# charlie-foxtrot/RTLSDR-Airband

Measured on NVIDIA H100. Metric: iq_msamples_per_s_fft_demod, higher is better.
Workload: dtype f32

## Files before the change

### rtlsdr-airband_b200/csrc/abg_internal.h

```cpp
#pragma once
#include <cuda_runtime.h>
#include <stdint.h>

#include <mutex>

struct AbgPerDeviceSize {
    std::mutex m;
    size_t v[64] = {};
    template <class F>
    cudaError_t ensure(size_t want, F&& apply) {
        int dev = 0;
        cudaGetDevice(&dev);
        dev &= 63;
        std::lock_guard<std::mutex> lock(m);
        if (want > v[dev]) {
            cudaError_t e = apply();
            if (e != cudaSuccess) return e;
            v[dev] = want;
        }
        return cudaSuccess;
    }
};

#define ABG_AGC_EXTRA 100
#define ABG_SQ_BUF 102
#define ABG_MAX_TONES 52

enum { SQ_CLOSED = 0, SQ_OPENING = 1, SQ_CLOSING = 2, SQ_LOW_SIGNAL_ABORT = 3, SQ_OPEN = 4 };

struct ChanParams {
    int32_t dev;
    int32_t modulation;
    int32_t needs_raw_iq, has_iq_outputs;
    uint32_t dm_dphi;
    float alpha, ampfactor;
    int32_t afc;
    int32_t notch_on;
    float nd0, nd1, nd2;
    int32_t lp_on;
    float lp_gain, lp_yc0, lp_yc1;
    int32_t ctcss_on;
    int32_t n_tones[2];
    int32_t window[2];
};

struct ChanState {
    float noise_floor;
    int32_t manual;
    float manual_level, normal_ratio, flappy_ratio, avg_cap;
    float pre_full, pre_capped, post_full, post_capped;
    float level_cache;
    int32_t using_post;
    int32_t next_state, cur_state, delay;
    uint32_t sample_count_mod16;
    int32_t low_signal_count;
    uint32_t recent_open_count, closed_sample_count;
    int32_t head;
    unsigned long long open_count, flappy_count;
    int32_t ct_enough[2], ct_count[2], ct_has_tone[2];
    unsigned long long ct_found[2], ct_not_found[2];
    float nx1, nx2, ny1, ny2;
    float lx1r, lx1i, lx2r, lx2i, ly1r, ly1i, ly2r, ly2i;
    float agcavgfast;
    uint32_t dm_phi;
    float pr, pj, prev_waveout;
    unsigned long long active_counter;
    int32_t axc_prev;
};

struct K1Dev {
    const unsigned char* raw;
    unsigned long long start_byte;
    int32_t n_frames;
    int32_t pos0;
    int32_t g0, n_channels;
    int32_t hop_bytes;
    int32_t sfmt;
    float2* spec;
    int32_t spec_first_pos;
    int32_t wave_batch;
};

struct K2Dev {
    int32_t n_batches;
    int32_t fft_size;
    const float2* spec;
};

struct K1Launch {
    int fft_size;
    int n_devices;
    int max_frames;
    int frames_per_tile;
    int tile_bytes_cap;
    const K1Dev* devs;
    const int32_t* bins;
    const float* window_scaled;
    const float2* tw1;
    const float2* tw2;
    float* win;
    float2* iqin;
    int Gp;
    int sfmt;
};
cudaError_t abg_launch_k1(const K1Launch& L, cudaStream_t s);
int abg_k1_tile_frames(int fft_size, int sfmt, int hop_bytes, int* tile_bytes_cap);
cudaError_t abg_launch_k1_pruned(const K1Launch& L, const float2* twn, int max_channels, cudaStream_t s);
int abg_k1p_tile_frames(int fft_size, int sfmt, int hop_bytes, int max_channels, int* tile_bytes_cap);

struct K1TcPlan {
    int eligible;
    int K, HC, S, NC, ND, C2p, KBS, NSTB, acc_regs, smem_bytes, halo, consumer_warpgroups;
    int pps;
    size_t table_bytes;
};
struct K1TcTables {
    const int32_t* tab_of_dev;
    const signed char* btab;
    const long long* sq;
    int* counter;
    int32_t* status;
    double cscale;
};
int abg_k1tc_plan(int fft_size, int sfmt, int hop_bytes, int max_channels, int digits, K1TcPlan* p);
void abg_k1tc_build_table(const K1TcPlan& p, int fft_size, int sfmt, const float* wsc, const int32_t* bins, int n_channels, signed char* tab,
                          long long* sq, double* cscale);
cudaError_t abg_launch_k1_tc(const K1Launch& L, const K1TcPlan& p, const K1TcTables& T, int sm_count, cudaStream_t s);
int abg_k1tc_trace_dump(long long* out);

#define ABG_SPEC_FPC 32
struct SpecCfg {
    const float* wsc;
    float* partial;
    int32_t* counter;
    float* ring;
    int32_t hop_bytes, sfmt, stride, n_sel, n_chunks, ring_cap;
};
struct SpecRun {
    const unsigned char* raw;
    unsigned long long first_byte;
    int32_t n_batches;
    int32_t ring_pos0;
};
struct SpecArgs {
    const SpecCfg* cfg;
    const SpecRun* run;
    const float2* tw1;
    const float2* tw2;
    int wave_batch;
};
cudaError_t abg_launch_spectrum(int fft_size, const SpecArgs& a, int n_devices, int max_items, cudaStream_t s);

struct CarCfg {
    float* ring;
    int32_t g0, n_channels, ring_cap;
};
struct CarRun {
    int32_t n_batches;
    int32_t ring_pos0;
};
struct CarArgs {
    const CarCfg* cfg;
    const CarRun* run;
    const float2* iqin;
    int Gp, wave_batch;
};
cudaError_t abg_launch_carrier(const CarArgs& a, int n_devices, int max_items, cudaStream_t s);
int abg_carrier_items(int n_channels);

struct InmCfg {
    unsigned char* ring;
    uint32_t* hist;
    int32_t* counter;
    long long* partial;
    int32_t sfmt, hop_bytes, n_chunks, ring_cap;
    float scale;
};
#define ABG_INM_PARTIAL 6
struct InmRun {
    const unsigned char* raw;
    unsigned long long first_byte;
    int32_t n_batches;
    int32_t ring_pos0;
};
struct InmArgs {
    const InmCfg* cfg;
    const InmRun* run;
    int wave_batch;
};
cudaError_t abg_launch_input_meter(const InmArgs& a, int n_devices, int max_items, cudaStream_t s);
int abg_input_meter_chunks(int batch_bytes);

struct K2Launch {
    int G, Gp, P, wave_batch, fm_demod, iq_stride;
    int lanes_per_warp;
    int nfm_blocks;
    const ChanParams* params;
    ChanState* state;
    const K2Dev* devs;
    int32_t* bins;
    const int32_t* base_bins;
    float* win;
    float2* iqin;
    float* win_next;
    float2* iqin_next;
    float* wout;
    float2* iqout;
    float* sqbuf;
    const float* tone_coeff;
    float* tone_q1;
    float* tone_q2;
    float* tone_mag;
    unsigned char* axc;
    const float* sincos_lut;
};
cudaError_t abg_launch_k2(const K2Launch& L, cudaStream_t s);
int abg_k2_stats_dump(unsigned long long* out);

struct MixInput {
    int32_t g;
    int32_t dev;
    float mult_l, mult_r;
};
struct MixLaunch {
    int n_mixers, n_batches, wave_batch, P, Gp;
    const int32_t* offsets;
    const MixInput* inputs;
    const K2Dev* devs;
    const float* wout;
    const unsigned char* axc;
    float* sums;
    int32_t* flags;
    float* host_sums;
    int32_t* host_flags;
};
cudaError_t abg_launch_mix(const MixLaunch& L, cudaStream_t s);
struct K2Export {
    float* host_wout;
    float2* host_iqout;
    unsigned char* host_axc;
    size_t stride;
};
cudaError_t abg_launch_k2_tail(const K2Launch& L, const K2Export& X, cudaStream_t s);
```

### rtlsdr-airband_b200/csrc/k1_tc.cu

```cuda
#include <cuda_runtime.h>
#include <math.h>
#include <stdint.h>
#include <stdlib.h>

#include <algorithm>

#include "../../include/airband_b200.h"
#include "abg_internal.h"
#include "tc_ptx.cuh"

namespace {
using namespace tc;
extern long long* g_tc_trace;

constexpr int TC_THREADS = 384;
constexpr int TC_A_THREADS = 96;
constexpr int TC_CONSUMER_WARPS = 8;
constexpr int TC_CTRL_BYTES = 1024;
constexpr int TC_MAX_STAGES = 32;
constexpr int TC_INFO_SLOTS = 4;

struct TileInfo {
    const unsigned char* src;
    int nf;
    int pos;
    int gbase;
    int nch;
    int tab;
    int pad;
};

struct TcArgs {
    const K1Dev* devs;
    const int32_t* tab_of_dev;
    const signed char* btab;
    const long long* sq;
    float* win;
    float2* iqin;
    int* counter;
    int32_t* status;
    double cscale;
    int Gp, n_devices, tiles_per_dev, total_tiles;
    int K, hop_bytes, S, npairs;
    int KBS, NSTG, pps;
    int a_bytes, stage_bytes;
    long long* trace;
};

struct Ctrl {
    unsigned long long full[TC_MAX_STAGES], empty[TC_MAX_STAGES];
    unsigned long long info_full[TC_INFO_SLOTS], info_empty[TC_INFO_SLOTS];
    TileInfo info[TC_INFO_SLOTS];
};
static_assert(sizeof(Ctrl) <= TC_CTRL_BYTES, "control block too large");

struct StageSeq {
    int p, np, q0, nq, nk, sh, mk;
    __device__ __forceinline__ void start(const TcArgs& a) {
        nk = (a.K - 32 * p + a.hop_bytes - 1) / a.hop_bytes;
        q0 = 0;
        nq = min(a.KBS, nk);
        np = min(min(a.pps, a.npairs - p), ((a.K - (nk - 1) * a.hop_bytes + 31) >> 5) - p);
        sh = np > 1 ? nq - 1 : 31;
        mk = np > 1 ? nq - 1 : -1;
    }
    __device__ __forceinline__ void first(const TcArgs& a) {
        p = 0;
        start(a);
    }
    __device__ __forceinline__ bool next(const TcArgs& a) {
        q0 += nq;
        if (q0 < nk) {
            nq = min(a.KBS, nk - q0);
            return true;
        }
        p += np;
        if (p >= a.npairs) return false;
        start(a);
        return true;
    }
};

template <int ND, int C2P, bool S8, bool GROUPED>
__global__ void __launch_bounds__(TC_THREADS, 1) k1_tc_kernel(const TcArgs a) {
    constexpr int NCOL = (ND * C2P + 31) & ~31;
    constexpr int KSTEP_BYTES = NCOL * 32;
    extern __shared__ __align__(1024) unsigned char smem[];
    Ctrl* c = reinterpret_cast<Ctrl*>(smem);
    const uint32_t ring = smem_u32(smem + TC_CTRL_BYTES);
    const uint32_t full0 = smem_u32(&c->full[0]), empty0 = smem_u32(&c->empty[0]);
    const int tid = threadIdx.x, lane = tid & 31;
    const int warp = __shfl_sync(0xffffffffu, tid >> 5, 0);

    if (tid == 0) {
        for (int i = 0; i < TC_MAX_STAGES; i++) {
            mbar_init(smem_u32(&c->full[i]), TC_A_THREADS + 1);
            mbar_init(smem_u32(&c->empty[i]), TC_CONSUMER_WARPS);
        }
        for (int i = 0; i < TC_INFO_SLOTS; i++) {
            mbar_init(smem_u32(&c->info_full[i]), 1);
            mbar_init(smem_u32(&c->info_empty[i]), TC_CONSUMER_WARPS);
        }
        fence_mbar_init();
    }
    __syncthreads();

#define TC_TRACE_STAGE(role, it, st, e)                                                                          \
    do {                                                                                                         \
        if (a.trace && (it) == 3 && (st) < 16) a.trace[((size_t)blockIdx.x * 4 + (role)) * 64 + 32 + 2 * (st) + (e)] = clock64(); \
    } while (0)
#define TC_TRACE(role, it, ev)                                                                                   \
    do {                                                                                                         \
        if (a.trace && (it) < 8 && (threadIdx.x & 31) == 0) a.trace[(((size_t)blockIdx.x * 4 + (role)) * 16 + (it)) * 4 + (ev)] = clock64(); \
    } while (0)
    if (warp < 3) {
        const int rr = tid & 7;
        uint32_t stg = 0, ph = 0;
        for (int it = 0;; ++it) {
            const int slot = it & (TC_INFO_SLOTS - 1);
            mbar_wait_spin(smem_u32(&c->info_full[slot]), (it / TC_INFO_SLOTS) & 1);
            const TileInfo ti = c->info[slot];
            if (ti.nf <= 0) break;
            if (warp == 0) TC_TRACE(0, it, 0);
            const int valid = (ti.nf - 1) * a.hop_bytes + a.K;
            StageSeq u;
            u.first(a);
            do {
                mbar_wait_spin(empty0 + 8 * stg, ph ^ 1);
                const int first = u.q0 * a.hop_bytes + 32 * u.p;
                const unsigned char* src = ti.src + first;
                const int rem = valid - first, nrows = 127 + u.nq, ncol = 2 * u.np;
                const uint32_t dst = ring + stg * (uint32_t)a.stage_bytes;
                const int total = ((nrows + 7) >> 3) * 8 * ncol;
                for (int i = tid; i - tid < total; i += TC_A_THREADS) {
                    const int u8 = i >> 3, rb = u8 / ncol, c = u8 - rb * ncol, r = rb * 8 + rr, off = r * a.hop_bytes + 16 * c;
                    if (i < total && r < nrows && off < rem) cp_async16(dst + c * a.S + r * 16, src + off);
                }
                cp_async_arrive_noinc(full0 + 8 * stg);
                if (++stg == (uint32_t)a.NSTG) stg = 0, ph ^= 1;
            } while (u.next(a));
            if (warp == 0) TC_TRACE(0, it, 3);
        }
    } else if (warp == 3) {
        const uint32_t leader = elect_one();
        const size_t tab_bytes = (size_t)a.K * NCOL;
        const int ks_per_row = a.hop_bytes / 32;
        auto publish = [&](int it) -> int {
            const int slot = it & (TC_INFO_SLOTS - 1);
            mbar_wait_spin(smem_u32(&c->info_empty[slot]), ((it / TC_INFO_SLOTS) & 1) ^ 1);
            TileInfo ti{};
            ti.nf = 0;
            ti.tab = -1;
            for (;;) {
                const int t = atomicAdd(a.counter, 1);
                if (t >= a.total_tiles) break;
                const int dev = t / a.tiles_per_dev, st = t - dev * a.tiles_per_dev;
                const K1Dev dv = a.devs[dev];
                const int f0 = st * 128;
                if (f0 >= dv.n_frames || dv.n_channels <= 0) continue;
                ti.src = dv.raw + dv.start_byte + (unsigned long long)f0 * dv.hop_bytes;
                ti.nf = min(128, dv.n_frames - f0);
                ti.pos = dv.pos0 + f0;
                ti.gbase = dv.g0;
                ti.nch = dv.n_channels;
                ti.tab = a.tab_of_dev[dev];
                break;
            }
            c->info[slot] = ti;
            mbar_arrive(smem_u32(&c->info_full[slot]));
            return ti.tab;
        };
        uint32_t stg = 0, ph = 0;
        int tab = lane == 0 ? publish(0) : 0;
        tab = __shfl_sync(0xffffffffu, tab, 0);
        for (int it = 0; tab >= 0; ++it) {
            int next_tab = lane == 0 ? publish(it + 1) : 0;
            next_tab = __shfl_sync(0xffffffffu, next_tab, 0);
            const signed char* src = a.btab + (size_t)tab * tab_bytes;
            TC_TRACE(2, it, 0);
            StageSeq u;
            u.first(a);
            int st = 0;
            do {
                mbar_wait_spin(empty0 + 8 * stg, ph ^ 1);
                TC_TRACE_STAGE(2, it, st, 0);
                if (leader) {
                    const uint32_t bar = full0 + 8 * stg, dst = ring + stg * (uint32_t)a.stage_bytes + (uint32_t)a.a_bytes;
                    mbar_arrive_expect_tx(bar, (uint32_t)(u.np * u.nq * KSTEP_BYTES));
                    for (int g = 0; g < u.np; g++)
                        for (int q = 0; q < u.nq; q++)
                            bulk_g2s(dst + (g * u.nq + q) * KSTEP_BYTES, src + (size_t)((u.q0 + q) * ks_per_row + u.p + g) * KSTEP_BYTES,
                                     (uint32_t)KSTEP_BYTES, bar);
                }
                TC_TRACE_STAGE(2, it, st, 1);
                st++;
                if (++stg == (uint32_t)a.NSTG) stg = 0, ph ^= 1;
            } while (u.next(a));
            TC_TRACE(2, it, 1);
            tab = next_tab;
        }
    } else if (warp >= 4) {
        const int wg = (warp - 4) >> 2;
        const int wq = warp & 3;
        uint32_t acc[NCOL / 2];
        const uint64_t adesc0 = smem_desc_noswizzle(0, (uint32_t)a.S, 128u), bdesc0 = smem_desc_noswizzle(0, (uint32_t)NCOL * 16u, 128u);
        const uint64_t a_hi = adesc0 >> 32 << 32, b_hi = bdesc0 >> 32 << 32;
        const uint32_t a_lo0 = (uint32_t)adesc0 + (ring >> 4) + (uint32_t)(wg * 64);
        const uint32_t b_lo0 = (uint32_t)bdesc0 + ((ring + (uint32_t)a.a_bytes) >> 4);
        const uint32_t stage16 = (uint32_t)a.stage_bytes >> 4, pair16 = (uint32_t)a.S >> 3;
        uint32_t stg = 0, ph = 0, prev_empty = 0;
        for (int it = 0;; ++it) {
            const int slot = it & (TC_INFO_SLOTS - 1);
            mbar_wait_spin(smem_u32(&c->info_full[slot]), (it / TC_INFO_SLOTS) & 1);
            const TileInfo ti = c->info[slot];
            if (ti.nf <= 0) break;
            if (warp == 4) TC_TRACE(3, it, 0);
            StageSeq u;
            u.first(a);
            uint32_t accumulate = 0;
            int st = 0;
            wgmma_fence_regs(acc);
            do {
                mbar_wait_spin(full0 + 8 * stg, ph);
                fence_proxy_async();
                if (warp == 4) TC_TRACE_STAGE(3, it, st, 0);
                const uint32_t a_lo = a_lo0 + stg * stage16, b_lo = b_lo0 + stg * stage16;
                const int n_mma = GROUPED ? u.np * u.nq : u.nq;
                for (int j = 0; j < n_mma; j++) {
                    const uint32_t a_off = GROUPED ? (uint32_t)(j >> u.sh) * pair16 + (uint32_t)(j & u.mk) : (uint32_t)j;
                    wgmma_fence_regs(acc);
                    wgmma_fence();
                    WgmmaI8<NCOL, S8>::mma(acc, a_hi | (a_lo + a_off), b_hi | (b_lo + j * (KSTEP_BYTES >> 4)), accumulate);
                    wgmma_commit();
                    wgmma_fence_regs(acc);
                    accumulate = 1;
                }
                wgmma_wait_groups(n_mma);
                mbar_arrive_if(prev_empty, st > 0 && lane == 0);
                prev_empty = empty0 + 8 * stg;
                if (warp == 4) TC_TRACE_STAGE(3, it, st, 1);
                st++;
                if (++stg == (uint32_t)a.NSTG) stg = 0, ph ^= 1;
            } while (u.next(a));
            wgmma_wait<0>();
            wgmma_fence_regs(acc);
            if (lane == 0) mbar_arrive(prev_empty);
            if (warp == 4) TC_TRACE(1, it, 1);
            constexpr long long MUL = S8 ? 1 : 2, OFF = S8 ? 0 : 255;
            const int r0 = wg * 64 + wq * 16 + (lane >> 2);
            const long long* sq = a.sq + (size_t)ti.tab * C2P;
#pragma unroll
            for (int jb = 0; jb < C2P / 8; jb++) {
                const int ch = 4 * jb + (lane & 3);
                const long long sq_re = __ldg(sq + 2 * ch), sq_im = __ldg(sq + 2 * ch + 1);
#pragma unroll
                for (int h = 0; h < 2; h++) {
                    long long v[2];
#pragma unroll
                    for (int e = 0; e < 2; e++) {
                        v[e] = 0;
#pragma unroll
                        for (int d = 0; d < ND; d++) v[e] = (v[e] << 8) + (long long)(int32_t)acc[4 * (d * C2P / 8 + jb) + 2 * h + e];
                    }
                    const float xr = (float)((double)(MUL * v[0] - OFF * sq_re) * a.cscale);
                    const float xi = (float)((double)(MUL * v[1] - OFF * sq_im) * a.cscale);
                    const int row = r0 + 8 * h;
                    if (row < ti.nf && ch < ti.nch) {
                        const size_t o = (size_t)(ti.pos + row) * a.Gp + ti.gbase + ch;
                        a.win[o] = sqrtf(__fadd_rn(__fmul_rn(xr, xr), __fmul_rn(xi, xi)));
                        a.iqin[o] = make_float2(xr, xi);
                    }
                }
            }
            __syncwarp();
            if (lane == 0) mbar_arrive(smem_u32(&c->info_empty[slot]));
            if (warp == 4) TC_TRACE(1, it, 2);
        }
    }
}

template <int ND, int C2P, bool S8>
cudaError_t tc_launch_one(const TcArgs& args, int grid, size_t smem, cudaStream_t s) {
    auto kern = args.pps > 1 ? k1_tc_kernel<ND, C2P, S8, true> : k1_tc_kernel<ND, C2P, S8, false>;
    static AbgPerDeviceSize configured[2];
    cudaError_t e = configured[args.pps > 1].ensure(smem, [&]() {
        cudaError_t e2 = cudaFuncSetAttribute(kern, cudaFuncAttributeMaxDynamicSharedMemorySize, (int)smem);
        if (e2 != cudaSuccess) return e2;
        cudaFuncSetAttribute(kern, cudaFuncAttributePreferredSharedMemoryCarveout, cudaSharedmemCarveoutMaxShared);
        return cudaSuccess;
    });
    if (e != cudaSuccess) return e;
    kern<<<grid, TC_THREADS, smem, s>>>(args);
    return cudaGetLastError();
}
template <int ND, bool S8>
cudaError_t tc_launch_nd(const TcArgs& args, int C2p, int grid, size_t smem, cudaStream_t s) {
    switch (C2p) {
        case 8: return tc_launch_one<ND, 8, S8>(args, grid, smem, s);
        case 16: return tc_launch_one<ND, 16, S8>(args, grid, smem, s);
        case 24: return tc_launch_one<ND, 24, S8>(args, grid, smem, s);
        case 32: return tc_launch_one<ND, 32, S8>(args, grid, smem, s);
        case 40: return tc_launch_one<ND, 40, S8>(args, grid, smem, s);
        case 48: return tc_launch_one<ND, 48, S8>(args, grid, smem, s);
        case 56: return tc_launch_one<ND, 56, S8>(args, grid, smem, s);
        case 64: return tc_launch_one<ND, 64, S8>(args, grid, smem, s);
    }
    return cudaErrorInvalidValue;
}

long long* g_tc_trace = nullptr;
}

int abg_k1tc_trace_dump(long long* out) {
    if (!g_tc_trace) return -1;
    cudaDeviceSynchronize();
    return cudaMemcpy(out, g_tc_trace, sizeof(long long) * 256 * 4 * 16 * 4, cudaMemcpyDeviceToHost) == cudaSuccess ? 0 : -1;
}

int abg_k1tc_plan(int fft_size, int sfmt, int hop_bytes, int max_channels, int digits, K1TcPlan* p) {
    *p = K1TcPlan{};
    if (sfmt != ABG_SFMT_U8 && sfmt != ABG_SFMT_S8) return 0;
    if (hop_bytes % 32 != 0 || hop_bytes < 32) return 0;
    if (digits != 3 && digits != 4) return 0;
    const int K = fft_size * 2;
    const int HC = hop_bytes / 16;
    const int halo = (K - 32) / hop_bytes;
    int rows = 128 + halo;
    if ((rows & 1) == 0) rows++;
    const int S = rows * 16;
    const int C2p = (2 * max_channels + 7) & ~7;
    const int NC = (digits * C2p + 31) & ~31;
    if (NC > 256) return 0;
    if (K > 16384) return 0;
    const size_t kstep = (size_t)NC * 32;
    size_t cap = 200 * 1024;
    if (const char* ev = getenv("ABG_K1_TC_CAP_KB")) cap = std::min<size_t>(227, std::max(64, atoi(ev))) * 1024;
    int max_stages = TC_MAX_STAGES;
    if (const char* ev = getenv("ABG_K1_TC_STAGES")) max_stages = std::min(TC_MAX_STAGES, std::max(2, atoi(ev)));
    const size_t hard_cap = 227 * 1024;
    auto stage_bytes = [&](int pps, int kbs) { return (((size_t)2 * pps * S + 127) & ~(size_t)127) + (size_t)pps * kbs * kstep; };
    auto stages = [&](int pps, int kbs, size_t c) {
        return c > TC_CTRL_BYTES ? (int)std::min<size_t>(max_stages, (c - TC_CTRL_BYTES) / stage_bytes(pps, kbs)) : 0;
    };
    const int kq = (K + hop_bytes - 1) / hop_bytes, npairs = std::min(HC / 2, K / 32);
    int pps = kq <= 2 ? std::max(1, std::min(12 / kq, npairs)) : 1, kbs = kq;
    while (pps > 1 && stages(pps, kbs, cap) < 4) pps--;
    while (kbs > 1 && stages(pps, kbs, cap) < 4) kbs = (kbs + 1) / 2;
    int nst = stages(pps, kbs, cap);
    if (nst < 2) nst = stages(pps, kbs, hard_cap);
    if (nst < 2) return 0;
    p->pps = pps;
    p->eligible = 1; p->K = K; p->HC = HC; p->S = S; p->NC = NC; p->ND = digits; p->C2p = C2p; p->KBS = kbs; p->NSTB = nst;
    p->acc_regs = NC / 2;
    p->consumer_warpgroups = 2;
    p->smem_bytes = (int)(TC_CTRL_BYTES + (size_t)nst * stage_bytes(pps, kbs)); p->halo = halo;
    p->table_bytes = (size_t)K * NC;
    return 1;
}

void abg_k1tc_build_table(const K1TcPlan& p, int fft_size, int sfmt, const float* wsc, const int32_t* bins, int n_channels, signed char* tab,
                          long long* sq, double* cscale) {
    const int N = fft_size, K = p.K, NC = p.NC, ND = p.ND;
    double gmax = 0.0;
    for (int n = 0; n < N; n++) gmax = std::max(gmax, fabs((double)wsc[n]));
    if (gmax <= 0.0) gmax = 1.0;
    const double Q = ldexp(1.0, 8 * ND - 2);
    std::fill(tab, tab + (size_t)K * NC, (signed char)0);
    for (int o = 0; o < p.C2p; o++) sq[o] = 0;
    for (int c = 0; c < n_channels; c++) {
        const int b = bins[c] & (N - 1);
        for (int n = 0; n < N; n++) {
            const double th = 2.0 * M_PI * (double)(((long long)n * b) % N) / (double)N;
            const double w = (double)wsc[n], cs = cos(th) * w, sn = sin(th) * w;
            const double coef[2][2] = {{cs, sn}, {-sn, cs}};
            for (int reim = 0; reim < 2; reim++)
                for (int comp = 0; comp < 2; comp++) {
                    const int o = 2 * c + reim;
                    const int kk = 2 * n + comp;
                    long long q = llround(coef[reim][comp] / gmax * Q);
                    sq[o] += q;
                    const int ks = kk >> 5, h = (kk >> 4) & 1, t = kk & 15;
                    for (int d = ND - 1; d >= 0; d--) {
                        long long dig = ((q + 128) & 255) - 128;
                        q = (q - dig) >> 8;
                        tab[((size_t)(ks * 2 + h) * NC + (size_t)(d * p.C2p + o)) * 16 + t] = (signed char)dig;
                    }
                }
        }
    }
    *cscale = (sfmt == ABG_SFMT_U8) ? gmax / (2.0 * Q) : gmax / Q;
}

cudaError_t abg_launch_k1_tc(const K1Launch& L, const K1TcPlan& p, const K1TcTables& T, int sm_count, cudaStream_t s) {
    TcArgs a{};
    a.devs = L.devs; a.tab_of_dev = T.tab_of_dev; a.btab = T.btab; a.sq = T.sq; a.win = L.win; a.iqin = L.iqin; a.counter = T.counter;
    a.status = T.status; a.cscale = T.cscale; a.Gp = L.Gp; a.n_devices = L.n_devices;
    a.tiles_per_dev = (L.max_frames + 127) / 128;
    a.total_tiles = a.tiles_per_dev * L.n_devices;
    a.K = p.K; a.hop_bytes = p.HC * 16; a.S = p.S; a.npairs = std::min(p.HC / 2, p.K / 32);
    a.KBS = p.KBS; a.NSTG = p.NSTB;
    a.pps = p.pps;
    a.a_bytes = (2 * p.pps * p.S + 127) & ~127;
    a.stage_bytes = a.a_bytes + p.pps * p.KBS * p.NC * 32;
    a.trace = nullptr;
    static long long* trace_buf = nullptr;
    if (getenv("ABG_K1_TC_TRACE")) {
        if (!trace_buf) {
            cudaMalloc((void**)&trace_buf, sizeof(long long) * 256 * 4 * 16 * 4);
            cudaMemset(trace_buf, 0, sizeof(long long) * 256 * 4 * 16 * 4);
        }
        a.trace = trace_buf;
        g_tc_trace = trace_buf;
    }
    if (a.total_tiles <= 0) return cudaSuccess;
    const int grid = std::min(a.total_tiles, std::max(sm_count, 1));
    const bool s8 = L.sfmt == ABG_SFMT_S8;
    const size_t smem = (size_t)p.smem_bytes;
    if (p.ND == 3) return s8 ? tc_launch_nd<3, true>(a, p.C2p, grid, smem, s) : tc_launch_nd<3, false>(a, p.C2p, grid, smem, s);
    if (p.ND == 4) return s8 ? tc_launch_nd<4, true>(a, p.C2p, grid, smem, s) : tc_launch_nd<4, false>(a, p.C2p, grid, smem, s);
    return cudaErrorInvalidValue;
}
```

Baseline: 258,100.

## Double M-tile to 256 frames per CTA for narrow ungrouped tensor-core K1

```diff
diff --git a/rtlsdr-airband_b200/csrc/abg_internal.h b/rtlsdr-airband_b200/csrc/abg_internal.h
--- a/rtlsdr-airband_b200/csrc/abg_internal.h
+++ b/rtlsdr-airband_b200/csrc/abg_internal.h
@@ -112,6 +112,7 @@
     int eligible;
     int K, HC, S, NC, ND, C2p, KBS, NSTB, acc_regs, smem_bytes, halo, consumer_warpgroups;
     int pps;
+    int tile_frames;
     size_t table_bytes;
 };
 struct K1TcTables {
diff --git a/rtlsdr-airband_b200/csrc/k1_tc.cu b/rtlsdr-airband_b200/csrc/k1_tc.cu
--- a/rtlsdr-airband_b200/csrc/k1_tc.cu
+++ b/rtlsdr-airband_b200/csrc/k1_tc.cu
@@ -19,6 +19,8 @@
 constexpr int TC_CTRL_BYTES = 1024;
 constexpr int TC_MAX_STAGES = 32;
 constexpr int TC_INFO_SLOTS = 4;
+
+__host__ __device__ constexpr int tc_tile_blocks(int ncol, bool grouped) { return (!grouped && ncol <= 64) ? 2 : 1; }
 
 struct TileInfo {
     const unsigned char* src;
@@ -85,6 +87,7 @@
 __global__ void __launch_bounds__(TC_THREADS, 1) k1_tc_kernel(const TcArgs a) {
     constexpr int NCOL = (ND * C2P + 31) & ~31;
     constexpr int KSTEP_BYTES = NCOL * 32;
+    constexpr int MB = tc_tile_blocks(NCOL, GROUPED), TILE = 128 * MB;
     extern __shared__ __align__(1024) unsigned char smem[];
     Ctrl* c = reinterpret_cast<Ctrl*>(smem);
     const uint32_t ring = smem_u32(smem + TC_CTRL_BYTES);
@@ -129,7 +132,7 @@
                 mbar_wait_spin(empty0 + 8 * stg, ph ^ 1);
                 const int first = u.q0 * a.hop_bytes + 32 * u.p;
                 const unsigned char* src = ti.src + first;
-                const int rem = valid - first, nrows = 127 + u.nq, ncol = 2 * u.np;
+                const int rem = valid - first, nrows = TILE - 1 + u.nq, ncol = 2 * u.np;
                 const uint32_t dst = ring + stg * (uint32_t)a.stage_bytes;
                 const int total = ((nrows + 7) >> 3) * 8 * ncol;
                 for (int i = tid; i - tid < total; i += TC_A_THREADS) {
@@ -156,10 +159,10 @@
                 if (t >= a.total_tiles) break;
                 const int dev = t / a.tiles_per_dev, st = t - dev * a.tiles_per_dev;
                 const K1Dev dv = a.devs[dev];
-                const int f0 = st * 128;
+                const int f0 = st * TILE;
                 if (f0 >= dv.n_frames || dv.n_channels <= 0) continue;
                 ti.src = dv.raw + dv.start_byte + (unsigned long long)f0 * dv.hop_bytes;
-                ti.nf = min(128, dv.n_frames - f0);
+                ti.nf = min(TILE, dv.n_frames - f0);
                 ti.pos = dv.pos0 + f0;
                 ti.gbase = dv.g0;
                 ti.nch = dv.n_channels;
@@ -202,10 +205,10 @@
     } else if (warp >= 4) {
         const int wg = (warp - 4) >> 2;
         const int wq = warp & 3;
-        uint32_t acc[NCOL / 2];
+        uint32_t acc[MB][NCOL / 2];
         const uint64_t adesc0 = smem_desc_noswizzle(0, (uint32_t)a.S, 128u), bdesc0 = smem_desc_noswizzle(0, (uint32_t)NCOL * 16u, 128u);
         const uint64_t a_hi = adesc0 >> 32 << 32, b_hi = bdesc0 >> 32 << 32;
-        const uint32_t a_lo0 = (uint32_t)adesc0 + (ring >> 4) + (uint32_t)(wg * 64);
+        const uint32_t a_lo0 = (uint32_t)adesc0 + (ring >> 4) + (uint32_t)(wg * 64 * MB);
         const uint32_t b_lo0 = (uint32_t)bdesc0 + ((ring + (uint32_t)a.a_bytes) >> 4);
         const uint32_t stage16 = (uint32_t)a.stage_bytes >> 4, pair16 = (uint32_t)a.S >> 3;
         uint32_t stg = 0, ph = 0, prev_empty = 0;
@@ -219,7 +222,8 @@
             u.first(a);
             uint32_t accumulate = 0;
             int st = 0;
-            wgmma_fence_regs(acc);
+#pragma unroll
+            for (int b = 0; b < MB; b++) wgmma_fence_regs(acc[b]);
             do {
                 mbar_wait_spin(full0 + 8 * stg, ph);
                 fence_proxy_async();
@@ -228,11 +232,15 @@
                 const int n_mma = GROUPED ? u.np * u.nq : u.nq;
                 for (int j = 0; j < n_mma; j++) {
                     const uint32_t a_off = GROUPED ? (uint32_t)(j >> u.sh) * pair16 + (uint32_t)(j & u.mk) : (uint32_t)j;
-                    wgmma_fence_regs(acc);
+                    const uint64_t bd = b_hi | (b_lo + j * (KSTEP_BYTES >> 4));
+#pragma unroll
+                    for (int b = 0; b < MB; b++) wgmma_fence_regs(acc[b]);
                     wgmma_fence();
-                    WgmmaI8<NCOL, S8>::mma(acc, a_hi | (a_lo + a_off), b_hi | (b_lo + j * (KSTEP_BYTES >> 4)), accumulate);
+#pragma unroll
+                    for (int b = 0; b < MB; b++) WgmmaI8<NCOL, S8>::mma(acc[b], a_hi | (a_lo + a_off + 64u * b), bd, accumulate);
                     wgmma_commit();
-                    wgmma_fence_regs(acc);
+#pragma unroll
+                    for (int b = 0; b < MB; b++) wgmma_fence_regs(acc[b]);
                     accumulate = 1;
                 }
                 wgmma_wait_groups(n_mma);
@@ -243,32 +251,36 @@
                 if (++stg == (uint32_t)a.NSTG) stg = 0, ph ^= 1;
             } while (u.next(a));
             wgmma_wait<0>();
-            wgmma_fence_regs(acc);
+#pragma unroll
+            for (int b = 0; b < MB; b++) wgmma_fence_regs(acc[b]);
             if (lane == 0) mbar_arrive(prev_empty);
             if (warp == 4) TC_TRACE(1, it, 1);
             constexpr long long MUL = S8 ? 1 : 2, OFF = S8 ? 0 : 255;
-            const int r0 = wg * 64 + wq * 16 + (lane >> 2);
             const long long* sq = a.sq + (size_t)ti.tab * C2P;
 #pragma unroll
-            for (int jb = 0; jb < C2P / 8; jb++) {
-                const int ch = 4 * jb + (lane & 3);
-                const long long sq_re = __ldg(sq + 2 * ch), sq_im = __ldg(sq + 2 * ch + 1);
-#pragma unroll
-                for (int h = 0; h < 2; h++) {
-                    long long v[2];
-#pragma unroll
-                    for (int e = 0; e < 2; e++) {
-                        v[e] = 0;
-#pragma unroll
-                        for (int d = 0; d < ND; d++) v[e] = (v[e] << 8) + (long long)(int32_t)acc[4 * (d * C2P / 8 + jb) + 2 * h + e];
-                    }
-                    const float xr = (float)((double)(MUL * v[0] - OFF * sq_re) * a.cscale);
-                    const float xi = (float)((double)(MUL * v[1] - OFF * sq_im) * a.cscale);
-                    const int row = r0 + 8 * h;
-                    if (row < ti.nf && ch < ti.nch) {
-                        const size_t o = (size_t)(ti.pos + row) * a.Gp + ti.gbase + ch;
-                        a.win[o] = sqrtf(__fadd_rn(__fmul_rn(xr, xr), __fmul_rn(xi, xi)));
-                        a.iqin[o] = make_float2(xr, xi);
+            for (int b = 0; b < MB; b++) {
+                const int r0 = (wg * MB + b) * 64 + wq * 16 + (lane >> 2);
+#pragma unroll
+                for (int jb = 0; jb < C2P / 8; jb++) {
+                    const int ch = 4 * jb + (lane & 3);
+                    const long long sq_re = __ldg(sq + 2 * ch), sq_im = __ldg(sq + 2 * ch + 1);
+#pragma unroll
+                    for (int h = 0; h < 2; h++) {
+                        long long v[2];
+#pragma unroll
+                        for (int e = 0; e < 2; e++) {
+                            v[e] = 0;
+#pragma unroll
+                            for (int d = 0; d < ND; d++) v[e] = (v[e] << 8) + (long long)(int32_t)acc[b][4 * (d * C2P / 8 + jb) + 2 * h + e];
+                        }
+                        const float xr = (float)((double)(MUL * v[0] - OFF * sq_re) * a.cscale);
+                        const float xi = (float)((double)(MUL * v[1] - OFF * sq_im) * a.cscale);
+                        const int row = r0 + 8 * h;
+                        if (row < ti.nf && ch < ti.nch) {
+                            const size_t o = (size_t)(ti.pos + row) * a.Gp + ti.gbase + ch;
+                            a.win[o] = sqrtf(__fadd_rn(__fmul_rn(xr, xr), __fmul_rn(xi, xi)));
+                            a.iqin[o] = make_float2(xr, xi);
+                        }
                     }
                 }
             }
@@ -325,9 +337,6 @@
     const int K = fft_size * 2;
     const int HC = hop_bytes / 16;
     const int halo = (K - 32) / hop_bytes;
-    int rows = 128 + halo;
-    if ((rows & 1) == 0) rows++;
-    const int S = rows * 16;
     const int C2p = (2 * max_channels + 7) & ~7;
     const int NC = (digits * C2p + 31) & ~31;
     if (NC > 256) return 0;
@@ -338,18 +347,28 @@
     int max_stages = TC_MAX_STAGES;
     if (const char* ev = getenv("ABG_K1_TC_STAGES")) max_stages = std::min(TC_MAX_STAGES, std::max(2, atoi(ev)));
     const size_t hard_cap = 227 * 1024;
+    int mb = 1, S = 0;
+    auto set_tile = [&](int blocks) {
+        mb = blocks;
+        int rows = 128 * mb + halo;
+        if ((rows & 1) == 0) rows++;
+        S = rows * 16;
+    };
     auto stage_bytes = [&](int pps, int kbs) { return (((size_t)2 * pps * S + 127) & ~(size_t)127) + (size_t)pps * kbs * kstep; };
     auto stages = [&](int pps, int kbs, size_t c) {
         return c > TC_CTRL_BYTES ? (int)std::min<size_t>(max_stages, (c - TC_CTRL_BYTES) / stage_bytes(pps, kbs)) : 0;
     };
     const int kq = (K + hop_bytes - 1) / hop_bytes, npairs = std::min(HC / 2, K / 32);
     int pps = kq <= 2 ? std::max(1, std::min(12 / kq, npairs)) : 1, kbs = kq;
+    set_tile(tc_tile_blocks(NC, pps > 1));
     while (pps > 1 && stages(pps, kbs, cap) < 4) pps--;
+    set_tile(tc_tile_blocks(NC, pps > 1));
     while (kbs > 1 && stages(pps, kbs, cap) < 4) kbs = (kbs + 1) / 2;
     int nst = stages(pps, kbs, cap);
     if (nst < 2) nst = stages(pps, kbs, hard_cap);
     if (nst < 2) return 0;
     p->pps = pps;
+    p->tile_frames = 128 * mb;
     p->eligible = 1; p->K = K; p->HC = HC; p->S = S; p->NC = NC; p->ND = digits; p->C2p = C2p; p->KBS = kbs; p->NSTB = nst;
     p->acc_regs = NC / 2;
     p->consumer_warpgroups = 2;
@@ -395,7 +414,7 @@
     TcArgs a{};
     a.devs = L.devs; a.tab_of_dev = T.tab_of_dev; a.btab = T.btab; a.sq = T.sq; a.win = L.win; a.iqin = L.iqin; a.counter = T.counter;
     a.status = T.status; a.cscale = T.cscale; a.Gp = L.Gp; a.n_devices = L.n_devices;
-    a.tiles_per_dev = (L.max_frames + 127) / 128;
+    a.tiles_per_dev = (L.max_frames + p.tile_frames - 1) / p.tile_frames;
     a.total_tiles = a.tiles_per_dev * L.n_devices;
     a.K = p.K; a.hop_bytes = p.HC * 16; a.S = p.S; a.npairs = std::min(p.HC / 2, p.K / 32);
     a.KBS = p.KBS; a.NSTG = p.NSTB;
```

Measured after the change: 264,600 (median of 6 runs). +2.5%, better.
